# UBC-AWP/vision-sam3-yolo-lameless

Measured on AMD Instinct MI355X. Metric: frames/sec (whole node) for YOLO+SAM3+DINOv3 feature extraction, 1080p clips, higher is better.
Workload: dtype f16; 1 GPU; BASELINE cfg#5, dense schedule: fused per-frame path on a synthetic 5 s @ 30 fps 1080p clip (150 unique BGR frames resident in HBM): YOLOv8-l detect (letterbox 384x640, NMS, scale_boxes; f16 plan) -> SAM (Hiera-B+ image encoder + FPN at 1024x1024, box-prompted mask decoder, 1080p mask + statistics + contour features) + DINOv3 ViT-L/16 embed (224x224) on EVERY frame; per-frame records packed, gathe; parallelism=one clip per GPU, 1 GPU(s), one gather per step, streams=7

## Files before the change

include/lmx.h:

```cpp
#ifndef LMX_H
#define LMX_H
#include <stdint.h>
#ifdef __cplusplus
extern "C" {
#endif

#define LMX_VERSION 100

#define LMX_OK 0
#define LMX_EINVAL (-1)
#define LMX_EHIP (-2)

typedef void* lmx_stream_t;

int lmx_version(void);
const char* lmx_last_error(void);
int lmx_device_count(void);

enum { LMX_F16 = 0, LMX_F32 = 1 };
enum { LMX_ACT_NONE = 0, LMX_ACT_SILU = 1, LMX_ACT_GELU = 2 , LMX_ACT_RELU = 3,
       LMX_ACT_SWIGLU = 4  };

typedef struct {
  const void* A;
// ... 94 lines not shown
                   lmx_stream_t stream);
int lmx_k_upsample2(const void* src, int64_t lds, void* dst, int64_t ldd, int n, int H, int W, int C,
                    lmx_stream_t stream);
int lmx_k_detect_decode(const float* head, int64_t ldh, float* pred, int n, int H, int W, int nc, float stride,
                        int a_off, int A, lmx_stream_t stream);
int lmx_k_scale_boxes(float* boxes, int total, float padx, float pady, float gain, float w, float h,
                      lmx_stream_t stream);

int lmx_k_split3(const float* x, int64_t ldx, int act, const void* res3, int64_t ldr, void* out3, int64_t ldo, int64_t rows,
                 int N, int g, int nsum, int64_t sum_stride, lmx_stream_t stream);
int lmx_k_maxpool5_x3(const void* src3, int64_t lds, void* dst3, int64_t ldd, int n, int H, int W, int C, lmx_stream_t stream);
int lmx_k_stem_conv_x3(const uint8_t* img, const float* w, const float* bias, void* out3, int n, int H, int W, int Cout,
                       lmx_stream_t stream);
int lmx_k_attention_f32(const float* q, int64_t ldq, const float* k, int64_t ldk, const float* v, int64_t ldv, float* o,
                        int64_t ldo, int B, int H, int Tq, int Tk, int hd, float scale, lmx_stream_t stream);
int lmx_k_hyper_mask_f32(const float* up, const float* hyper, float* logits, int n, int G, int C, int act, lmx_stream_t stream);

int lmx_k_pose_gather(const float* raw0, const float* raw1, const float* raw2, int64_t ldk, const int32_t* hw,
                      const float* strides, const int32_t* src, const int32_t* counts, int n, int max_det, int K, int ndim,
                      float padx, float pady, float gain, float w, float h, float* out, lmx_stream_t stream);

int lmx_k_im2col_u8(const uint8_t* img, const float* lut, void* out, int n, int rh, int rw, int IH, int IW, int KH,
                    int KW, int stride, int pad, int64_t ldo, lmx_stream_t stream);
int lmx_k_maxpool2(const void* src, int64_t lds, void* dst, int64_t ldd, int dtype, int n, int H, int W, int C,
                   lmx_stream_t stream);
int lmx_k_cast_f32_f16(const float* src, int64_t lds, void* dst, int64_t ldd, int64_t rows, int cols,
                       lmx_stream_t stream);
int lmx_h_hiera_band(const int* window, const int* q_stride, int n_blocks, int grid, int nh, int nw, int* band);
int lmx_k_band_join(const void* band, const void* table, void* out, int dtype, int n, int H, int Hb, int W, int D,
                    lmx_stream_t stream);

int lmx_k_add_bcast(const void* a, int a_dtype, int64_t lda, const float* b, int64_t ldb, int b_rows, void* out,
                    int out_dtype, int64_t ldo, int64_t rows, int D, lmx_stream_t stream);
int lmx_k_prompt_box(const float* boxes, int64_t ldb, float* sparse, int n, double sx, double sy, float S,
                     const float* gauss, const float* corner, int F, lmx_stream_t stream);
int lmx_k_hyper_mask(const void* up, const float* hyper, float* logits, int n, int G, int C, lmx_stream_t stream);
int lmx_k_mask_post(const float* logits, int n, int L, int T, int nh, int nw, int h, int w, uint8_t* mask,
                    int64_t* stats, float* workspace, lmx_stream_t stream);
int lmx_k_prompt_points(const float* points, const int32_t* labels, int Np, const float* boxes, int64_t ldb, float* sparse, int n,
                        double sx, double sy, float S, const float* gauss, const float* point_embed, const float* not_a_point,
                        const float* corner, int F, lmx_stream_t stream);
#define LMX_MASK_EMBED_PARAMS 4684
int lmx_k_mask_embed(const float* mask_input, const void* emb, int emb_dtype, int64_t lde, const float* params, float* keys,
                     int64_t ldk, int n, int G, lmx_stream_t stream);
int lmx_k_hyper_mask_multi(const void* up, const float* hyper, float* logits, int n, int M, int G, int C, lmx_stream_t stream);
int lmx_k_hyper_mask_multi_f32(const float* up, const float* hyper, float* logits, int n, int M, int G, int C, int act,
// ... 22 lines not shown
```

vision-sam3-yolo-lameless_amd/csrc/pre.hip:

```cpp
#include "common.h"

namespace {

constexpr int PRECISION_BITS = 32 - 8 - 2;

__device__ __forceinline__ uint8_t clip8(int v) {
  v >>= PRECISION_BITS;
  return (uint8_t)(v < 0 ? 0 : (v > 255 ? 255 : v));
}

constexpr int RESIZE_H_MAX_ROW = 16384;
__global__ __launch_bounds__(256) void pil_resize_h_kernel(const uint8_t* __restrict__ src, uint8_t* __restrict__ dst,
                                                           int n, int sh, int sw, int dw,
                                                           const int32_t* __restrict__ bounds,
                                                           const int32_t* __restrict__ kk, int ksize, int swap_rb) {
  __shared__ __attribute__((aligned(16))) uint8_t rowbuf[RESIZE_H_MAX_ROW];
  const int rowb = sw * 3;
  for (int64_t row = blockIdx.x; row < (int64_t)n * sh; row += gridDim.x) {
    const uint8_t* srow = src + row * rowb;
    const int mis = (int)(reinterpret_cast<uintptr_t>(srow) & 15);
    const int head = mis ? 16 - mis : 0;
    for (int i = threadIdx.x; i < head && i < rowb; i += blockDim.x) rowbuf[i] = srow[i];
    const int nvec = (rowb - head) > 0 ? (rowb - head) / 16 : 0;
    for (int v = threadIdx.x; v < nvec; v += blockDim.x) {
      const u32x4 x = *reinterpret_cast<const u32x4*>(srow + head + v * 16);
      uint8_t* d = rowbuf + head + v * 16;
      if ((head & 3) == 0) {
        reinterpret_cast<unsigned*>(d)[0] = x[0];
        reinterpret_cast<unsigned*>(d)[1] = x[1];
        reinterpret_cast<unsigned*>(d)[2] = x[2];
        reinterpret_cast<unsigned*>(d)[3] = x[3];
      } else {
#pragma unroll
        for (int e = 0; e < 16; ++e) d[e] = (uint8_t)(x[e >> 2] >> (8 * (e & 3)));
      }
    }
    for (int i = head + nvec * 16 + threadIdx.x; i < rowb; i += blockDim.x) rowbuf[i] = srow[i];
    __syncthreads();
    uint8_t* drow = dst + row * dw * 3;
    for (int xo = threadIdx.x; xo < dw; xo += blockDim.x) {
      const int xmin = bounds[2 * xo], cnt = bounds[2 * xo + 1];
      const int32_t* k = kk + (int64_t)xo * ksize;
      const uint8_t* s = rowbuf + xmin * 3;
      int a0 = 1 << (PRECISION_BITS - 1), a1 = a0, a2 = a0;
      for (int x = 0; x < cnt; ++x) {
        const int c = k[x];
        a0 += (int)s[3 * x + 0] * c;
        a1 += (int)s[3 * x + 1] * c;
        a2 += (int)s[3 * x + 2] * c;
      }
      uint8_t* d = drow + xo * 3;
      if (swap_rb) {
        d[0] = clip8(a2);
        d[1] = clip8(a1);
        d[2] = clip8(a0);
      } else {
        d[0] = clip8(a0);
        d[1] = clip8(a1);
        d[2] = clip8(a2);
      }
    }
    __syncthreads();
  }
}

__global__ __launch_bounds__(256) void pil_resize_v_kernel(const uint8_t* __restrict__ src, uint8_t* __restrict__ dst,
                                                           int n, int sh, int dh, int w,
                                                           const int32_t* __restrict__ bounds,
                                                           const int32_t* __restrict__ kk, int ksize) {
  const int rowb = w * 3;
  const int64_t total = (int64_t)n * dh * rowb;
  for (int64_t i = (int64_t)blockIdx.x * blockDim.x + threadIdx.x; i < total; i += (int64_t)gridDim.x * blockDim.x) {
    const int xb = (int)(i % rowb);
    const int64_t r = i / rowb;
    const int yo = (int)(r % dh);
    const int img = (int)(r / dh);
    const int ymin = bounds[2 * yo], cnt = bounds[2 * yo + 1];
    const int32_t* k = kk + (int64_t)yo * ksize;
    const uint8_t* s = src + ((int64_t)img * sh + ymin) * rowb + xb;
    int a = 1 << (PRECISION_BITS - 1);
    for (int y = 0; y < cnt; ++y) a += (int)s[(int64_t)y * rowb] * k[y];
    dst[i] = clip8(a);
// ... 154 lines not shown
    if (yo >= dh) break;
    const int py = yo / P, ky = yo - py * P;
    half_t* d = out + (((int64_t)img * gh + py) * gw + px) * ldo + (ky * P + kxp) * 3;
    d[0] = (half_t)(((swap_rb ? acc[r][2] : acc[r][0]) - m0) / s0);
    d[1] = (half_t)((acc[r][1] - m1) / s1);
    d[2] = (half_t)(((swap_rb ? acc[r][0] : acc[r][2]) - m2) / s2);
  }
}

inline int grid_for(int64_t total) {
  int64_t g = (total + 255) / 256;
  if (g > 256 * 8) g = 256 * 8;
  if (g < 1) g = 1;
  return (int)g;
}

}

extern "C" int lmx_k_pil_resize_h(const uint8_t* src, uint8_t* dst, int n, int sh, int sw, int dw, const int32_t* bounds,
                                  const int32_t* kk, int ksize, int swap_rb, lmx_stream_t stream) {
  LMX_REQUIRE(src && dst && bounds && kk, "lmx_k_pil_resize_h: null pointer");
  LMX_REQUIRE(n > 0 && sh > 0 && sw > 0 && dw > 0 && ksize > 0, "lmx_k_pil_resize_h: shape");
  LMX_REQUIRE(sw * 3 <= RESIZE_H_MAX_ROW, "lmx_k_pil_resize_h: source rows wider than %d pixels are not staged", RESIZE_H_MAX_ROW / 3);
  int64_t rows = (int64_t)n * sh;
  hipLaunchKernelGGL(pil_resize_h_kernel, dim3((unsigned)(rows < 256 * 16 ? rows : 256 * 16)), dim3(256), 0,
                     reinterpret_cast<hipStream_t>(stream), src, dst, n, sh, sw, dw, bounds, kk, ksize, swap_rb);
  return lmx_launch_check("pil_resize_h_kernel");
}

extern "C" int lmx_k_pil_resize_v(const uint8_t* src, uint8_t* dst, int n, int sh, int dh, int w, const int32_t* bounds,
                                  const int32_t* kk, int ksize, lmx_stream_t stream) {
  LMX_REQUIRE(src && dst && bounds && kk, "lmx_k_pil_resize_v: null pointer");
  LMX_REQUIRE(n > 0 && sh > 0 && dh > 0 && w > 0 && ksize > 0, "lmx_k_pil_resize_v: shape");
  if ((w * 3) % 4 == 0 && (((uintptr_t)src | (uintptr_t)dst) & 3) == 0) {
    hipLaunchKernelGGL(pil_resize_v4_kernel, dim3(grid_for((int64_t)n * dh * (w * 3 / 4))), dim3(256), 0,
                       reinterpret_cast<hipStream_t>(stream), src, dst, n, sh, dh, w, bounds, kk, ksize);
    return lmx_launch_check("pil_resize_v4_kernel");
  }
  hipLaunchKernelGGL(pil_resize_v_kernel, dim3(grid_for((int64_t)n * dh * w * 3)), dim3(256), 0,
                     reinterpret_cast<hipStream_t>(stream), src, dst, n, sh, dh, w, bounds, kk, ksize);
  return lmx_launch_check("pil_resize_v_kernel");
}

extern "C" int lmx_k_float_resize_patchify(const uint8_t* src, void* out, int n, int sh, int sw, int gh, int gw, int P,
                                           int64_t ldo, const int32_t* bounds_h, const float* kk_h, int ksize_h,
                                           const int32_t* bounds_v, const float* kk_v, int ksize_v, int seg_cols,
                                           float rescale, const float* mean_std, int swap_rb, lmx_stream_t stream) {
  LMX_REQUIRE(src && out && bounds_h && kk_h && bounds_v && kk_v && mean_std, "lmx_k_float_resize_patchify: null pointer");
  LMX_REQUIRE(n > 0 && n <= 65535 && sh > 0 && sw > 0 && gh > 0 && gw > 0 && P > 0 && ksize_h > 0 && ksize_v > 0,
// ... 27 lines not shown
```

vision-sam3-yolo-lameless_amd/lmx/_lib.py:

```python
import ctypes as C
import os

_HERE = os.path.dirname(os.path.abspath(__file__))
LIB_PATH = os.environ.get("LMX_LIB") or os.path.join(_HERE, "liblmx.so")


class LmxError(RuntimeError):
    pass


class GemmDesc(C.Structure):
    _fields_ = [
        ("A", C.c_void_p), ("W", C.c_void_p), ("bias", C.c_void_p), ("scale", C.c_void_p), ("res", C.c_void_p),
        ("C", C.c_void_p),
        ("lda", C.c_int64), ("ldc", C.c_int64), ("ldr", C.c_int64),
        ("M", C.c_int32), ("N", C.c_int32), ("K", C.c_int32),
        ("act", C.c_int32), ("out_dtype", C.c_int32), ("a_mode", C.c_int32),
        ("H", C.c_int32), ("W_", C.c_int32), ("Cin", C.c_int32), ("conv_stride", C.c_int32),
        ("Ho", C.c_int32), ("Wo", C.c_int32), ("res_rows", C.c_int32), ("a_rep", C.c_int32), ("split_k", C.c_int32), ("split_stride", C.c_int64),
        ("ln_out", C.c_void_p), ("ln_gamma", C.c_void_p), ("ln_beta", C.c_void_p), ("ld_ln", C.c_int64), ("ln_eps", C.c_float),
    ]


class AttnDesc(C.Structure):
# ... 30 lines not shown
    "lmx_k_relpos_tables": (_I, [C.POINTER(AttnDesc), _VP, _VP, _I, _VP, _VP]),
    "lmx_k_rope": (_I, [_VP, _I64, _I, _I, _I, _I, _I, _VP, _VP, _VP]),
    "lmx_k_pil_resize_h": (_I, [_VP, _VP, _I, _I, _I, _I, _VP, _VP, _I, _I, _VP]),
    "lmx_k_pil_resize_v": (_I, [_VP, _VP, _I, _I, _I, _I, _VP, _VP, _I, _VP]),
    "lmx_k_patchify_norm": (_I, [_VP, _VP, _I, _I, _I, _I, _I, _I, _I, _I, _I64, _VP, _VP]),
    "lmx_k_float_resize_patchify": (_I, [_VP, _VP, _I, _I, _I, _I, _I, _I, _I64, _VP, _VP, _I, _VP, _VP, _I, _I, _F, _VP, _I, _VP]),
    "lmx_k_assemble_tokens": (_I, [_VP, _VP, _VP, _VP, _I, _I, _I, _I, _VP]),
    "lmx_k_token_mean": (_I, [_VP, _I, _VP, _I, _I, _I, _VP]),
    "lmx_k_swiglu": (_I, [_VP, _I64, _VP, _I64, _I, _I, _VP]),
    "lmx_nms_workspace_bytes": (_I64, [_I, _I]),
    "lmx_k_nms": (_I, [_VP, _I, _I, _I, _F, _D, _I, _F, _VP, _VP, _VP, _VP, _VP, _VP, _VP]),
    "lmx_k_letterbox": (_I, [_VP, _VP, _I, _I, _I, _I, _I, _I, _I, _I, _I, _VP, _VP, _VP, _VP, _I, _VP]),
    "lmx_k_stem_conv": (_I, [_VP, _VP, _VP, _VP, _I, _I, _I, _I, _VP]),
    "lmx_k_split3": (_I, [_VP, _I64, _I, _VP, _I64, _VP, _I64, _I64, _I, _I, _I, _I64, _VP]),
    "lmx_k_maxpool5_x3": (_I, [_VP, _I64, _VP, _I64, _I, _I, _I, _I, _VP]),
    "lmx_k_stem_conv_x3": (_I, [_VP, _VP, _VP, _VP, _I, _I, _I, _I, _VP]),
    "lmx_k_attention_f32": (_I, [_VP, _I64, _VP, _I64, _VP, _I64, _VP, _I64, _I, _I, _I, _I, _I, _F, _VP]),
    "lmx_k_hyper_mask_f32": (_I, [_VP, _VP, _VP, _I, _I, _I, _I, _VP]),
    "lmx_k_maxpool5": (_I, [_VP, _I64, _VP, _I64, _I, _I, _I, _I, _VP]),
    "lmx_k_upsample2": (_I, [_VP, _I64, _VP, _I64, _I, _I, _I, _I, _VP]),
    "lmx_k_detect_decode": (_I, [_VP, _I64, _VP, _I, _I, _I, _I, _F, _I, _I, _VP]),
    "lmx_k_scale_boxes": (_I, [_VP, _I, _F, _F, _F, _F, _F, _VP]),
    "lmx_k_im2col_u8": (_I, [_VP, _VP, _VP, _I, _I, _I, _I, _I, _I, _I, _I, _I, _I64, _VP]),
    "lmx_k_maxpool2": (_I, [_VP, _I64, _VP, _I64, _I, _I, _I, _I, _I, _VP]),
    "lmx_k_cast_f32_f16": (_I, [_VP, _I64, _VP, _I64, _I64, _I, _VP]),
    "lmx_h_hiera_band": (_I, [C.POINTER(C.c_int), C.POINTER(C.c_int), _I, _I, _I, _I, C.POINTER(C.c_int)]),
    "lmx_k_band_join": (_I, [_VP, _VP, _VP, _I, _I, _I, _I, _I, _I, _VP]),
    "lmx_k_add_bcast":(_I, [_VP, _I, _I64, _VP, _I64, _I, _VP, _I, _I64, _I64, _I, _VP]),
    "lmx_h_mask_features": (_I, [_VP, _I, _I, _VP]),
    "lmx_h_iou_matrix": (_I, [_VP, _I, _VP, _I, _VP]),
    "lmx_h_assign": (_I, [_VP, _I, _I, _VP, _VP]),
    "lmx_contour_workspace_bytes": (_I64, [_I, _I, _I]),
    "lmx_k_contour_features": (_I, [_VP, _I, _I, _I, _VP, _VP, _VP]),
    "lmx_k_prompt_box": (_I, [_VP, _I64, _VP, _I, _D, _D, _F, _VP, _VP, _I, _VP]),
    "lmx_k_hyper_mask": (_I, [_VP, _VP, _VP, _I, _I, _I, _VP]),
    "lmx_k_mask_post": (_I, [_VP, _I, _I, _I, _I, _I, _I, _I, _VP, _VP, _VP, _VP]),
    "lmx_k_prompt_points": (_I, [_VP, _VP, _I, _VP, _I64, _VP, _I, _D, _D, _F, _VP, _VP, _VP, _VP, _I, _VP]),
    "lmx_k_mask_embed": (_I, [_VP, _VP, _I, _I64, _VP, _VP, _I64, _I, _I, _VP]),
    "lmx_k_hyper_mask_multi": (_I, [_VP, _VP, _VP, _I, _I, _I, _I, _VP]),
    "lmx_k_hyper_mask_multi_f32": (_I, [_VP, _VP, _VP, _I, _I, _I, _I, _I, _VP]),
    "lmx_k_mask_logits": (_I, [_VP, _I, _I, _I, _I, _I, _I, _I, _VP, _VP]),
    "lmx_k_mask_score": (_I, [_VP, _I, _I, _I, _I, _I, _I, _I, _D, _D, _VP, _VP, _VP]),
    "lmx_k_nms_boxes": (_I, [_VP, _I64, _VP, _VP, _I, _D, _VP, _VP, _VP, _VP]),
}

_lib = None
# ... 26 lines not shown
```

vision-sam3-yolo-lameless_amd/lmx/kernels.py:

```python
import ctypes as C
import os
import threading

import torch

from . import _lib
from ._lib import AttnDesc, GemmDesc, LmxError, check

F16, F32 = 0, 1
ACT_NONE, ACT_SILU, ACT_GELU, ACT_RELU, ACT_SWIGLU = 0, 1, 2, 3, 4
_DT = {torch.float16: F16, torch.float32: F32}


_tls = threading.local()


def _stream(dev):
    _tls.dev = dev
    return C.c_void_p(torch.cuda.current_stream(dev).cuda_stream)


def _ptr(t):
    return C.c_void_p(t.data_ptr()) if t is not None else C.c_void_p(0)

# ... 129 lines not shown
        h, g, b, eps = ln_out
        Mh, Nh, ldh = _rows(h, "gemm ln_out")
        if (Mh, Nh) != (Mout, Nout) or h.dtype != torch.float16:
            raise LmxError(f"gemm: ln_out must be float16 [{Mout},{Nout}], got {h.dtype} {tuple(h.shape)}")
        if any(t.dtype != torch.float32 or t.numel() != Nout or not t.is_contiguous() for t in (g, b)):
            raise LmxError("gemm: ln_out's gamma and beta must be contiguous float32 [N]")
        d.ln_out, d.ln_gamma, d.ln_beta, d.ld_ln, d.ln_eps = h.data_ptr(), g.data_ptr(), b.data_ptr(), ldh, float(eps)
    check(_lib.load().lmx_k_gemm(C.byref(d), _stream(dev)), "lmx_k_gemm")
    return out


def im2col_u8(img, lut, IH, IW, KH, KW, stride, pad, ldo):
    dev = _dev(img, lut)
    n, rh, rw, c = img.shape
    if c != 3 or img.dtype != torch.uint8 or not img.is_contiguous():
        raise LmxError("im2col_u8: img must be contiguous uint8 [n,h,w,3]")
    OH, OW = (IH + 2 * pad - KH) // stride + 1, (IW + 2 * pad - KW) // stride + 1
    out = torch.empty((n * OH * OW, ldo), dtype=torch.float16, device=img.device)
    check(_lib.load().lmx_k_im2col_u8(_ptr(img), _ptr(lut), _ptr(out), n, rh, rw, IH, IW, KH, KW, stride, pad, ldo,
                                      _stream(dev)), "lmx_k_im2col_u8")
    return out


def maxpool2(x, out):
    dev = _dev(x, out)
    n, H, W, Cc, ps = _nhwc(x, "maxpool2 x")
    no, Ho, Wo, Co, pso = _nhwc(out, "maxpool2 out")
    if (no, Ho, Wo, Co) != (n, H // 2, W // 2, Cc) or x.dtype != out.dtype:
        raise LmxError("maxpool2: shape/dtype mismatch")
    check(_lib.load().lmx_k_maxpool2(_ptr(x), ps, _ptr(out), pso, _DT[x.dtype], n, H, W, Cc, _stream(dev)), "lmx_k_maxpool2")
    return out


def cast_f16(x, out=None):
    dev = _dev(x, out)
    rows, cols, lds = _rows(x, "cast src")
    if out is None:
        out = torch.empty((rows, cols), dtype=torch.float16, device=x.device)
    check(_lib.load().lmx_k_cast_f32_f16(_ptr(x), lds, _ptr(out), out.stride(0), rows, cols, _stream(dev)),
          "lmx_k_cast_f32_f16")
    return out


def hiera_band(windows, q_strides, grid, nh, nw):
    nb = len(windows)
    if nb != len(q_strides):
# ... 703 lines not shown
    out = torch.empty((n, 8), dtype=torch.int64, device=mask.device)
    check(lib.lmx_k_contour_features(_ptr(mask), n, h, w, _ptr(out), _ptr(ws), _stream(dev)), "lmx_k_contour_features")
    return out


LAUNCH_TRACE = None
_raw_lib = None
RIDGE_FLOP_PER_BYTE = 2500e12 / 8e12


def _work(name, args):
    if name == "lmx_k_gemm":
        d = args[0]._obj
        M, N, Kd = d.M, d.N, d.K
        osz = 4 if d.out_dtype == F32 else 2
        a_bytes = 2 * M * (Kd // max(d.a_rep, 1))
        if d.a_mode == 1:
            a_bytes = 2 * (M // max(d.Ho * d.Wo, 1)) * d.H * d.W_ * d.Cin
        by = a_bytes + 2 * N * Kd + osz * (M // 4 if d.a_mode == 2 else M) * (N // 2 if d.act == ACT_SWIGLU else N) + (osz * (d.res_rows or M) * N if d.res else 0)
        by += 2 * M * N if d.ln_out else 0
        fl = 2.0 * M * N * Kd
        key = f"gemm M={M} N={N} K={Kd} out={'f32' if osz == 4 else 'f16'} conv3x3={d.a_mode} act={d.act} res={int(bool(d.res))}" + (" ln_out" if d.ln_out else "")
        return ("gemm/mfma-bound" if fl / by >= RIDGE_FLOP_PER_BYTE else "gemm/hbm-bound"), fl, by, key
    if name == "lmx_k_attention":
        d = args[0]._obj
        fl = 4.0 * d.B * d.H * d.Tq * d.Tk * d.hd
        by = 2 * d.H * d.hd * d.B * (2 * d.Tq + 2 * d.Tk)
        key = f"attention B={d.B} H={d.H} Tq={d.Tq} Tk={d.Tk} hd={d.hd} mode={d.mode} ws={d.ws} qs={d.q_stride} rel={int(bool(d.rel))}"
        return ("attention/mfma-bound" if fl / by >= RIDGE_FLOP_PER_BYTE else "attention/hbm-bound"), fl, by, key
    if name == "lmx_k_layernorm":
        in_dt, out_dt, rows, D = args[1], args[6], args[8], args[9]
        return "layernorm", 0.0, rows * D * ((4 if in_dt == F32 else 2) + (4 if out_dt == F32 else 2)), f"layernorm rows={rows} D={D} in={in_dt} out={out_dt}"
    if name == "lmx_k_ln_mlp_img":
        rows, D = args[4], args[5]
        return "fused ln+mlp", 16.0 * D * D * rows, (8 + (2 if args[7] else 0) + (2 if args[8] else 0)) * D * rows, f"ln_mlp_img rows={rows} D={D}"
    if name == "lmx_k_ln_mlp":
        rows, D = args[8], args[9]
        return "fused ln+mlp", 16.0 * D * D * rows, (16 + (2 if args[12] else 0) + (2 if args[15] else 0)) * D * rows, f"ln_mlp rows={rows} D={D}"
    if name == "lmx_k_hiera_attn8":
        n_, Gh, Gw, D = args[10], args[11], args[12], args[13]
        rows = n_ * Gh * Gw
        return "fused attention half", rows * (8.0 * D * D + 256.0 * D), rows * D * (8 + (2 if args[0] else 0)), f"hiera_attn8 rows={rows} D={D} ln_inside={int(not args[0])}"
    if name == "lmx_k_hiera_attn4":
        n_, Gh, Gw, D = args[5], args[6], args[7], args[8]
        rows = n_ * Gh * Gw
        return "fused attention half", rows * (8.0 * D * D + 64.0 * D), rows * D * 10, f"hiera_attn4 rows={rows} D={D}"
# ... 80 lines not shown
```

vision-sam3-yolo-lameless_amd/lmx/sam.py:

```python
import math
import os
import threading
from dataclasses import dataclass

import numpy as np
import torch

from . import kernels as K
from . import resample

SAM_PIXEL_MEAN = (123.675, 116.28, 103.53)
SAM_PIXEL_STD = (58.395, 57.12, 57.375)


@dataclass
class HieraConfig:
    hidden: int = 112
    blocks: tuple = (2, 3, 16, 3)
    dims: tuple = (112, 224, 448, 896)
    heads: tuple = (2, 4, 8, 16)
    windows: tuple = (8, 4, 14, 7)
    global_blocks: tuple = (12, 16, 20)
    pos_bkg: tuple = (14, 14)
    q_pool_stages: int = 3
# ... 189 lines not shown
    kslot = np.array([16 * (2 * s_ + hb) + 4 * g + i for s_ in range(nks) for g in range(4) for hb in range(2) for i in range(4)])
    k15, k7 = (lambda r: r & 15), (lambda r: (r >> 1) & 7)
    imgs = []
    for ch in range(4 * D // 64):
        m1 = np.zeros((64, cols), np.float16)
        ok = kslot < D
        m1[:, ok] = w1[64 * ch: 64 * ch + 64][:, kslot[ok]].astype(np.float16)
        m2 = np.zeros((D, 64), np.float16)
        m2[:, :] = w2[:, 64 * ch + kslot[:64]].astype(np.float16)
        i1, i2 = _lds_image(m1, k15), _lds_image(m2, k7)
        if D <= 128:
            both = i1.copy()
            both[8192:8192 + D * 64] = i2[:D * 64]
            imgs.append(both)
        else:
            imgs += [i1, i2]
    z = np.zeros((D,), np.float32)
    bias = np.concatenate([b1, b2, g2, e2, gn if gn is not None else z, en if en is not None else z]).astype(np.float32)
    return np.stack(imgs), bias


class HieraEncoder:

    def __init__(self, cfg, state_dict, device="cuda", fused_mlp=True, band=True):
        self.cfg = cfg
        self.band = band
        self.device = torch.device(device)
        self.fused_mlp = fused_mlp and not os.environ.get("LMX_NO_FUSED_MLP")
        dev = self.device
        sd = state_dict

        def t32(a):
            return torch.from_numpy(np.ascontiguousarray(a, dtype=np.float32)).to(dev)

        def t16(a):
            return t32(a).to(torch.float16).contiguous()

        w = np.transpose(sd["backbone.patch_embed.projection.weight"], (0, 2, 3, 1)).reshape(cfg.hidden, 147)
        self.k_pad = 152
        self.pe_w = t16(np.concatenate([w, np.zeros((cfg.hidden, self.k_pad - 147), np.float32)], 1))
        self.pe_b = t32(sd["backbone.patch_embed.projection.bias"])
        g = cfg.image // 4
        pe = torch.nn.functional.interpolate(torch.from_numpy(sd["backbone.pos_embed"]), size=(g, g), mode="bicubic")
        win = torch.from_numpy(sd["backbone.pos_embed_window"])
        pe = pe + win.tile([x // y for x, y in zip(pe.shape, win.shape)])
        self.pos = pe.permute(0, 2, 3, 1).reshape(g * g, cfg.hidden).contiguous().to(dev)
        self.grid0 = g
        self.blocks = []
        for i, (dim, dim_out, heads, win_, qs) in enumerate(cfg.block_plan()):
# ... 41 lines not shown
        self._tabs = {}
        self.first_global = next((i for i, B in enumerate(self.blocks) if B["win"] == 0), None)
        self._bands, self._band_tabs, self._band_lock = {}, {}, threading.Lock()

    def _tables(self, h, w):
        key = (h, w)
        if key not in self._tabs:
            nh, nw = resize_longest_side(h, w, self.cfg.image)
            dev = self.device

            def up(tab):
                b, k, ks = tab
                return (torch.from_numpy(b).to(dev), torch.from_numpy(k).to(dev), ks)

            th = up(resample.coeff_tables(w, nw, resample.BILINEAR)) if nw != w else None
            tv = up(resample.coeff_tables(h, nh, resample.BILINEAR)) if nh != h else None
            self._tabs[key] = (nh, nw, th, tv)
        return self._tabs[key]

    def preprocess(self, frames, band=0):
        n, h, w, _ = frames.shape
        nh, nw, th, tv = self._tables(h, w)
        img = K.pil_resize(frames, nw, nh, th, tv, swap_rb=False)
        S = self.cfg.image
        return img, K.im2col_u8(img, self.lut, 4 * band if band else S, S, 7, 7, 4, 3, self.k_pad)

    def band_rows(self, nh, nw):
        if (nh, nw) not in self._bands:
            plan = self.cfg.block_plan()
            self._bands[(nh, nw)] = K.hiera_band([p[3] for p in plan], [p[4] for p in plan], self.grid0, nh, nw)
        return self._bands[(nh, nw)]

    def _selection(self):
        H = W = self.grid0
        sel = []
        for i, B in enumerate(self.blocks[:self.first_global]):
            dim, D, heads, win, qs = B["dim"], B["dim_out"], B["heads"], B["win"], B["qs"]
            sel.append((self._attn8(i, H, W), "attnp" in B and K.hiera_attn_pool_ok(dim, D, heads, win, H, W, qs),
                        "attn4" in B and K.hiera_attn4_ok(D, heads, win, H, W, qs), "mlp_img" in B and K.ln_mlp_img_ok(D, H * W)))
            if qs:
                H, W = H // 2, W // 2
        return tuple(sel)

    def _band_table(self, frames, nh, nw, band):
        key = (nh, nw, band, self._selection())
        tab = self._band_tabs.get(key)
        if tab is not None:
            return tab
        if torch.cuda.is_current_stream_capturing():
            raise K.LmxError("HieraEncoder: the constant rows below the band are not built for this frame geometry, and a stream capture "
                             "cannot build them (it needs a synchronisation): call encode() once before capturing")
        with self._band_lock:
            if key in self._band_tabs:
                return self._band_tabs[key]
            trace, K.LAUNCH_TRACE = K.LAUNCH_TRACE, None
            try:
                g = self.grid0
                x, H, W, stages, stages16 = self.trunk(self.preprocess(frames[:1])[1], 1, until=self.first_global)

                def below(t, Hs, Ws):
                    return t.reshape(Hs, Ws, -1)[band * Hs // g:].reshape(-1, t.shape[-1]).clone()

                tab = dict(x=below(x, H, W), stages=[below(s, *s.shape[1:3]) for s in stages],
                           stages16=[below(s16, *s.shape[1:3]) if s16 is not None else None for s, s16 in zip(stages, stages16)])
            finally:
                K.LAUNCH_TRACE = trace
            torch.cuda.current_stream(self.device).synchronize()
            self._band_tabs[key] = tab
        return tab

    def trunk(self, patches, n, band=0, table=None, lowest=0, until=None):
        cfg = self.cfg
        g = self.grid0
        H, W = band or g, g
        Hf = g
        x = K.gemm(patches, self.pe_w, bias=self.pe_b, res=self.pos[:H * g], res_rows=H * g, out_dtype=torch.float32)
        stage_ends = set(int(v) for v in np.cumsum(cfg.blocks) - 1)
        stages, stages16 = [], []
        dev = x.device
        h_next = None
        for i, B in enumerate(self.blocks):
            if i == until:
                return x, H, W, stages, stages16
            if band and i == self.first_global:
                x = K.band_join(x.view(n, H, W, -1), table["x"], Hf).view(n * Hf * W, -1)
                H, band, h_next = Hf, 0, None
            dim, D, heads, qs = B["dim"], B["dim_out"], B["heads"], B["qs"]
            rows = n * H * W
            h2 = None
            if self._attn8(i, H, W):
                if B["attn8_ln"]:
                    K.hiera_attn8(x, B["attn8"], n, H, W, heads, ln=(B["g1"], B["b1"], cfg.eps))
                else:
                    K.hiera_attn8(x, B["attn8"], n, H, W, heads, h=h_next if h_next is not None else K.layernorm(x, B["g1"], B["b1"], cfg.eps))
            elif "attnp" in B and K.hiera_attn_pool_ok(dim, D, heads, B["win"], H, W, qs):
                x = K.hiera_attn_pool(h_next if h_next is not None else K.layernorm(x, B["g1"], B["b1"], cfg.eps), B["attnp"], n, H, W, heads, D)
                H, W = H // 2, W // 2
            elif "attn4" in B and K.hiera_attn4_ok(D, heads, B["win"], H, W, qs):
                K.hiera_attn4(h_next if h_next is not None else K.layernorm(x, B["g1"], B["b1"], cfg.eps), x, B["attn4"], n, H, W, heads)
# ... 97 lines not shown
            if i not in cfg.fpn_top_down or i == nlev:
                K.gemm(a, w, bias=b, out=out.view(-1, cfg.fpn_dim))
            else:
                up = torch.empty((n, H, W, cfg.fpn_dim), dtype=torch.float16, device=s.device)
                K.upsample2(prev, up)
                K.gemm(a, w, bias=b, res=up.view(-1, cfg.fpn_dim), out=out.view(-1, cfg.fpn_dim))
            prev = out
            feats[i] = out
        return feats[:3]

    def encode_patches(self, patches, n):
        stages, stages16 = self.trunk(patches, n)
        return dict(fpn=self.fpn(stages, stages16), stages=stages)

    def encode(self, frames, precision=None, outputs="all"):
        if outputs not in ("all", "embedding"):
            raise ValueError(f"outputs {outputs!r}: expected 'all' or 'embedding'")
        lowest = 2 if outputs == "embedding" else 0
        n, h, w, _ = frames.shape
        nh, nw = self._tables(h, w)[:2]
        band = self.band_rows(nh, nw) if self.band else 0
        table = self._band_table(frames, nh, nw, band) if band else None
        img, patches = self.preprocess(frames, band)
        stages, stages16 = self.trunk(patches, n, band, table, lowest)
        return dict(fpn=self.fpn(stages, stages16, lowest), stages=stages, resized=img)


@dataclass
class SamVitConfig:
    hidden: int = 768
    layers: int = 12
    heads: int = 12
    mlp: int = 3072
    global_idx: tuple = (2, 5, 8, 11)
    window: int = 14
    patch: int = 16
    image: int = 1024
    out_ch: int = 256
    eps: float = 1e-6

    @property
    def grid(self):
        return self.image // self.patch


def sam_vit_b():
    return SamVitConfig()
# ... 160 lines not shown
```

Measured before the change: 788.2 frames/s.

## Fuse Hiera patch-embed im2col with GEMM and restructure horizontal resize kernel

Measured after the change: 794.0 frames/s (median of 6 runs). About the same (+0.7%).

```diff
diff --git a/include/lmx.h b/include/lmx.h
--- a/include/lmx.h
+++ b/include/lmx.h
@@ -140,6 +140,10 @@
 
 int lmx_k_im2col_u8(const uint8_t* img, const float* lut, void* out, int n, int rh, int rw, int IH, int IW, int KH,
                     int KW, int stride, int pad, int64_t ldo, lmx_stream_t stream);
+int lmx_h_patch_embed_ok(int N, int KH, int KW, int stride, int pad, int* ok);
+int lmx_k_patch_embed_u8(const uint8_t* img, const float* lut, const void* w, const float* bias, const float* res, int64_t ldr,
+                         int res_rows, float* out, int64_t ldc, int n, int rh, int rw, int IH, int IW, int N, int KH, int KW,
+                         int stride, int pad, lmx_stream_t stream);
 int lmx_k_maxpool2(const void* src, int64_t lds, void* dst, int64_t ldd, int dtype, int n, int H, int W, int C,
                    lmx_stream_t stream);
 int lmx_k_cast_f32_f16(const float* src, int64_t lds, void* dst, int64_t ldd, int64_t rows, int cols,
diff --git a/vision-sam3-yolo-lameless_amd/csrc/patch_embed.hip b/vision-sam3-yolo-lameless_amd/csrc/patch_embed.hip
--- /dev/null
+++ b/vision-sam3-yolo-lameless_amd/csrc/patch_embed.hip
@@ -0,0 +1,209 @@
+#include "common.h"
+
+namespace {
+
+constexpr int PE_TOK = 128;
+constexpr int PE_K = 147, PE_LDW = 152;
+constexpr int PE_RS = 168;
+constexpr int PE_ROW_BYTES = (4 * (PE_TOK - 1) + 7) * 3;
+constexpr int PE_P16 = 1554;
+constexpr int PE_LINES = (PE_ROW_BYTES + 15 + 15) / 16;
+constexpr int PE_PF = (7 * PE_LINES + 255) / 256;
+static_assert(PE_P16 >= PE_ROW_BYTES, "normalised row");
+
+struct PeTile {
+  int b, oy, tx0, ntok, y0, xs;
+  bool live;
+};
+__device__ __forceinline__ PeTile pe_tile(int tile, int tpr, int OH, int OW, int rh, int rw) {
+  PeTile t;
+  const int tx = tile % tpr, r = tile / tpr;
+  t.oy = r % OH;
+  t.b = r / OH;
+  t.tx0 = tx * PE_TOK;
+  t.ntok = OW - t.tx0 < PE_TOK ? OW - t.tx0 : PE_TOK;
+  t.y0 = 4 * t.oy - 3;
+  t.xs = 4 * t.tx0 - 3;
+  t.live = t.y0 < rh && t.xs < rw;
+  return t;
+}
+struct PeLine {
+  int ky;
+  intptr_t c0, L, g0, g1;
+  bool row_ok;
+};
+__device__ __forceinline__ PeLine pe_line(const PeTile& t, int item, const uint8_t* img, int rh, int rw) {
+  PeLine l;
+  l.ky = item % 7;
+  const int ci = item / 7;
+  const int y = t.y0 + l.ky;
+  l.row_ok = y >= 0 && y < rh;
+  const int x_lo = t.xs < 0 ? 0 : t.xs;
+  int x_hi = t.xs + 4 * (t.ntok - 1) + 7;
+  x_hi = x_hi < rw ? x_hi : rw;
+  const intptr_t rowp = reinterpret_cast<intptr_t>(img) + ((int64_t)t.b * rh + y) * rw * 3;
+  l.L = rowp + t.xs * 3;
+  l.g0 = rowp + x_lo * 3;
+  l.g1 = rowp + x_hi * 3;
+  l.c0 = (l.L & ~(intptr_t)15) + 16 * ci;
+  return l;
+}
+
+template <int NF>
+__global__ __launch_bounds__(256, 2) void patch_embed_u8_kernel(const uint8_t* __restrict__ img, const float* __restrict__ lut,
+                                                                const half_t* __restrict__ w, const float* __restrict__ bias,
+                                                                const float* __restrict__ res, int64_t ldr, int res_rows,
+                                                                float* __restrict__ out, int64_t ldc, int rh, int rw, int OH, int OW,
+                                                                int ntiles) {
+  __shared__ __attribute__((aligned(16))) half_t patch[PE_TOK * PE_RS];
+  __shared__ __attribute__((aligned(16))) half_t rows16[7 * PE_P16];
+  __shared__ half_t lut_s[768];
+  const int tid = threadIdx.x, lane = tid & 63;
+  const int wave = __builtin_amdgcn_readfirstlane(tid >> 6);
+  const int frow = lane & 15, fq = lane >> 4;
+  for (int i = tid; i < 768; i += 256) lut_s[i] = (half_t)lut[i];
+  for (int i = tid; i < PE_TOK * 3; i += 256) *reinterpret_cast<half8_t*>(patch + (i / 3) * PE_RS + 144 + (i % 3) * 8) = half8_t{0, 0, 0, 0, 0, 0, 0, 0};
+
+  half8_t wf[5][NF];
+#pragma unroll
+  for (int t = 0; t < 5; ++t)
+#pragma unroll
+    for (int j = 0; j < NF; ++j) {
+      const int k0 = 32 * t + 8 * fq;
+      wf[t][j] = half8_t{0, 0, 0, 0, 0, 0, 0, 0};
+      if (k0 < PE_LDW) wf[t][j] = *reinterpret_cast<const half8_t*>(w + (j * 16 + frow) * PE_LDW + k0);
+    }
+
+  const int tpr = (OW + PE_TOK - 1) / PE_TOK;
+  u32x4 pf[PE_PF];
+  auto request = [&](const PeTile& t) {
+    if (!t.live) return;
+#pragma unroll
+    for (int q = 0; q < PE_PF; ++q) {
+      const int item = tid + 256 * q;
+      pf[q] = u32x4{0, 0, 0, 0};
+      if (item < 7 * PE_LINES) {
+        const PeLine l = pe_line(t, item, img, rh, rw);
+        if (l.row_ok && l.c0 + 16 > l.g0 && l.c0 < l.g1) pf[q] = *reinterpret_cast<const u32x4*>(l.c0);
+      }
+    }
+  };
+  if ((int)blockIdx.x < ntiles) request(pe_tile(blockIdx.x, tpr, OH, OW, rh, rw));
+  for (int tile = blockIdx.x; tile < ntiles; tile += gridDim.x) {
+    const PeTile T = pe_tile(tile, tpr, OH, OW, rh, rw);
+    if (T.live) {
+#pragma unroll
+      for (int q = 0; q < PE_PF; ++q) {
+        const int item = tid + 256 * q;
+        if (item < 7 * PE_LINES) {
+          const PeLine l = pe_line(T, item, img, rh, rw);
+          const int i0 = (int)(l.c0 - l.L);
+          half_t* d = rows16 + l.ky * PE_P16;
+#pragma unroll
+          for (int e = 0; e < 16; ++e) {
+            const int i = i0 + e;
+            if (i >= 0 && i < PE_ROW_BYTES) {
+              const unsigned byte = (pf[q][e >> 2] >> (8 * (e & 3))) & 255u;
+              const bool in = l.row_ok && l.c0 + e >= l.g0 && l.c0 + e < l.g1;
+              d[i] = in ? lut_s[(i % 3) * 256 + byte] : (half_t)0.f;
+            }
+          }
+        }
+      }
+      __syncthreads();
+#pragma unroll
+      for (int it = 0; it < PE_TOK * 19 / 256 + 1; ++it) {
+        const int tok = tid & (PE_TOK - 1);
+        const int ck = __builtin_amdgcn_readfirstlane((it * 256 + tid) / PE_TOK);
+        if (ck < 19) {
+          half8_t v;
+#pragma unroll
+          for (int e = 0; e < 8; ++e) {
+            const int k = ck * 8 + e;
+            const int ky = k / 21, j = k - ky * 21;
+            v[e] = k < PE_K ? rows16[ky * PE_P16 + 12 * tok + j] : (half_t)0.f;
+          }
+          *reinterpret_cast<half8_t*>(patch + tok * PE_RS + ck * 8) = v;
+        }
+      }
+      __syncthreads();
+    }
+    if (tile + (int)gridDim.x < ntiles) request(pe_tile(tile + gridDim.x, tpr, OH, OW, rh, rw));
+    const int mbase = T.oy * OW + T.tx0;
+    const int rbase = res_rows > 0 ? (int)(((int64_t)T.b * OH * OW + mbase) % res_rows) : 0;
+#pragma unroll
+    for (int i = 0; i < 2; ++i) {
+      f32x4 acc[NF];
+#pragma unroll
+      for (int j = 0; j < NF; ++j) acc[j] = f32x4{0.f, 0.f, 0.f, 0.f};
+      const int tok = wave * 32 + i * 16 + frow;
+      if (T.live) {
+        const half_t* ap = patch + tok * PE_RS + fq * 8;
+        half8_t af[5];
+#pragma unroll
+        for (int t = 0; t < 5; ++t) af[t] = *reinterpret_cast<const half8_t*>(ap + 32 * t);
+#pragma unroll
+        for (int t = 0; t < 5; ++t)
+#pragma unroll
+          for (int j = 0; j < NF; ++j) acc[j] = __builtin_amdgcn_mfma_f32_16x16x32_f16(wf[t][j], af[t], acc[j], 0, 0, 0);
+      }
+      if (tok < T.ntok) {
+        const int64_t m = (int64_t)T.b * OH * OW + mbase + tok;
+        const int64_t mr = res_rows > 0 ? (int64_t)((rbase + tok) % res_rows) : m;
+        const float* rp = res + mr * ldr + fq * 4;
+        float* op = out + m * ldc + fq * 4;
+#pragma unroll
+        for (int j = 0; j < NF; ++j) {
+          f32x4 v = acc[j];
+          v += *reinterpret_cast<const f32x4*>(bias + j * 16 + fq * 4);
+          f32x4 o = v;
+          o += *reinterpret_cast<const f32x4*>(rp + j * 16);
+          *reinterpret_cast<f32x4*>(op + j * 16) = o;
+        }
+      }
+    }
+  }
+}
+
+template <int NF>
+int launch_patch_embed(const uint8_t* img, const float* lut, const void* w, const float* bias, const float* res, int64_t ldr,
+                       int res_rows, float* out, int64_t ldc, int rh, int rw, int OH, int OW, int ntiles, hipStream_t st) {
+  int dev;
+  LMX_TRY(lmx_stream_device(st, &dev));
+  const int cus = lmx_cu_count(dev);
+  if (cus < 0) return cus;
+  const int grid = ntiles < 2 * cus ? ntiles : 2 * cus;
+  hipLaunchKernelGGL(patch_embed_u8_kernel<NF>, dim3((unsigned)grid), dim3(256), 0, st, img, lut, reinterpret_cast<const half_t*>(w), bias,
+                     res, ldr, res_rows, out, ldc, rh, rw, OH, OW, ntiles);
+  return lmx_launch_check("patch_embed_u8_kernel");
+}
+
+}
+
+extern "C" int lmx_h_patch_embed_ok(int N, int KH, int KW, int stride, int pad, int* ok) {
+  LMX_REQUIRE(ok, "lmx_h_patch_embed_ok: null pointer");
+  *ok = KH == 7 && KW == 7 && stride == 4 && pad == 3 && N % 16 == 0 && N >= 96 && N <= 128;
+  return LMX_OK;
+}
+
+extern "C" int lmx_k_patch_embed_u8(const uint8_t* img, const float* lut, const void* w, const float* bias, const float* res, int64_t ldr,
+                                    int res_rows, float* out, int64_t ldc, int n, int rh, int rw, int IH, int IW, int N, int KH, int KW,
+                                    int stride, int pad, lmx_stream_t stream) {
+  LMX_REQUIRE(img && lut && w && bias && res && out, "lmx_k_patch_embed_u8: null pointer");
+  int ok = 0;
+  LMX_TRY(lmx_h_patch_embed_ok(N, KH, KW, stride, pad, &ok));
+  LMX_REQUIRE(ok, "lmx_k_patch_embed_u8: built for 7 x 7 / stride 4 / pad 3 and N = 96, 112, 128 (lmx_h_patch_embed_ok); got %d x %d / %d / %d, N=%d: "
+              "use lmx_k_im2col_u8 + lmx_k_gemm", KH, KW, stride, pad, N);
+  LMX_REQUIRE(n > 0 && rh > 0 && rw > 0 && rh <= IH && rw <= IW, "lmx_k_patch_embed_u8: geometry");
+  LMX_REQUIRE((int64_t)rh * rw * 3 < 0x7fffffffll, "lmx_k_patch_embed_u8: frame too large");
+  const int OH = (IH + 2 * pad - KH) / stride + 1, OW = (IW + 2 * pad - KW) / stride + 1;
+  const int64_t ntiles = (int64_t)n * OH * ((OW + PE_TOK - 1) / PE_TOK);
+  LMX_REQUIRE((int64_t)n * OH * OW < 0x7fffffffll && ntiles < 0x7fffffffll, "lmx_k_patch_embed_u8: too many tokens");
+  LMX_REQUIRE(res_rows >= 0 && ldr >= N && ldc >= N && ldr % 4 == 0 && ldc % 4 == 0, "lmx_k_patch_embed_u8: ldr=%lld ldc=%lld res_rows=%d",
+              (long long)ldr, (long long)ldc, res_rows);
+  LMX_REQUIRE(aligned16(w) && aligned16(bias) && aligned16(res) && aligned16(out), "lmx_k_patch_embed_u8: w, bias, res and out must be 16-byte aligned");
+  hipStream_t st = reinterpret_cast<hipStream_t>(stream);
+  if (N == 96) return launch_patch_embed<6>(img, lut, w, bias, res, ldr, res_rows, out, ldc, rh, rw, OH, OW, (int)ntiles, st);
+  if (N == 112) return launch_patch_embed<7>(img, lut, w, bias, res, ldr, res_rows, out, ldc, rh, rw, OH, OW, (int)ntiles, st);
+  return launch_patch_embed<8>(img, lut, w, bias, res, ldr, res_rows, out, ldc, rh, rw, OH, OW, (int)ntiles, st);
+}
diff --git a/vision-sam3-yolo-lameless_amd/csrc/pre.hip b/vision-sam3-yolo-lameless_amd/csrc/pre.hip
--- a/vision-sam3-yolo-lameless_amd/csrc/pre.hip
+++ b/vision-sam3-yolo-lameless_amd/csrc/pre.hip
@@ -10,54 +10,143 @@
 }
 
 constexpr int RESIZE_H_MAX_ROW = 16384;
-__global__ __launch_bounds__(256) void pil_resize_h_kernel(const uint8_t* __restrict__ src, uint8_t* __restrict__ dst,
+constexpr int RESIZE_H_SEG = 2048;
+constexpr int RESIZE_H_THREADS = 512;
+constexpr int RESIZE_H_ROWBUF = RESIZE_H_MAX_ROW + 48;
+constexpr int RESIZE_H_OUTBUF = RESIZE_H_SEG * 3 + 16;
+constexpr int RESIZE_H_TAB_MAX = 65536 - RESIZE_H_ROWBUF - RESIZE_H_OUTBUF;
+constexpr int RESIZE_H_PF = RESIZE_H_MAX_ROW / 16 / RESIZE_H_THREADS;
+
+template <bool FAST>
+__device__ __forceinline__ int resize_h_mul(unsigned byte, int c) {
+  return FAST ? __mul24((int)byte, c) : (int)byte * c;
+}
+template <bool FAST>
+__device__ __forceinline__ void resize_h_pixel(const uint8_t* rowbuf, int o, int cnt, const int32_t* k, int& a0, int& a1, int& a2) {
+  const unsigned* wp = reinterpret_cast<const unsigned*>(rowbuf + (o & ~3));
+  const unsigned sh = (unsigned)o & 3u;
+  for (int x = 0; x < cnt; x += 4, wp += 3) {
+    const unsigned r0 = wp[0], r1 = wp[1], r2 = wp[2], r3 = wp[3];
+    const unsigned w0 = __builtin_amdgcn_alignbyte(r1, r0, sh), w1 = __builtin_amdgcn_alignbyte(r2, r1, sh),
+                   w2 = __builtin_amdgcn_alignbyte(r3, r2, sh);
+    const int c0 = k[x];
+    const int c1 = x + 1 < cnt ? k[x + 1] : 0, c2 = x + 2 < cnt ? k[x + 2] : 0, c3 = x + 3 < cnt ? k[x + 3] : 0;
+    a0 += resize_h_mul<FAST>(w0 & 255u, c0);
+    a1 += resize_h_mul<FAST>((w0 >> 8) & 255u, c0);
+    a2 += resize_h_mul<FAST>((w0 >> 16) & 255u, c0);
+    a0 += resize_h_mul<FAST>(w0 >> 24, c1);
+    a1 += resize_h_mul<FAST>(w1 & 255u, c1);
+    a2 += resize_h_mul<FAST>((w1 >> 8) & 255u, c1);
+    a0 += resize_h_mul<FAST>((w1 >> 16) & 255u, c2);
+    a1 += resize_h_mul<FAST>(w1 >> 24, c2);
+    a2 += resize_h_mul<FAST>(w2 & 255u, c2);
+    a0 += resize_h_mul<FAST>((w2 >> 8) & 255u, c3);
+    a1 += resize_h_mul<FAST>((w2 >> 16) & 255u, c3);
+    a2 += resize_h_mul<FAST>(w2 >> 24, c3);
+  }
+}
+
+template <bool TAB>
+__global__ __launch_bounds__(RESIZE_H_THREADS) void pil_resize_h_kernel(const uint8_t* __restrict__ src, uint8_t* __restrict__ dst,
                                                            int n, int sh, int sw, int dw,
                                                            const int32_t* __restrict__ bounds,
                                                            const int32_t* __restrict__ kk, int ksize, int swap_rb) {
-  __shared__ __attribute__((aligned(16))) uint8_t rowbuf[RESIZE_H_MAX_ROW];
+  extern __shared__ __attribute__((aligned(16))) uint8_t resize_h_smem[];
+  uint8_t* rowbuf = resize_h_smem;
+  uint8_t* outbuf = resize_h_smem + RESIZE_H_ROWBUF;
+  const int32_t* bnd = bounds;
+  const int32_t* kks = kk;
+  bool fast = false;
+  if (TAB) {
+    int32_t* tab = reinterpret_cast<int32_t*>(resize_h_smem + RESIZE_H_ROWBUF + RESIZE_H_OUTBUF);
+    for (int i = threadIdx.x; i < 2 * dw; i += blockDim.x) tab[i] = bounds[i];
+    int wide = 0;
+    for (int i = threadIdx.x; i < dw * ksize; i += blockDim.x) {
+      const int c = kk[i];
+      tab[2 * dw + i] = c;
+      wide |= (unsigned)(c + (1 << 23)) >= (1u << 24);
+    }
+    bnd = tab;
+    kks = tab + 2 * dw;
+    fast = !__syncthreads_or(wide);
+  }
+  const int tid = threadIdx.x;
   const int rowb = sw * 3;
-  for (int64_t row = blockIdx.x; row < (int64_t)n * sh; row += gridDim.x) {
+  const int64_t rows = (int64_t)n * sh;
+  u32x4 pf[RESIZE_H_PF];
+  unsigned pfb = 0;
+  auto request = [&](int64_t row) {
     const uint8_t* srow = src + row * rowb;
     const int mis = (int)(reinterpret_cast<uintptr_t>(srow) & 15);
-    const int head = mis ? 16 - mis : 0;
-    for (int i = threadIdx.x; i < head && i < rowb; i += blockDim.x) rowbuf[i] = srow[i];
-    const int nvec = (rowb - head) > 0 ? (rowb - head) / 16 : 0;
-    for (int v = threadIdx.x; v < nvec; v += blockDim.x) {
-      const u32x4 x = *reinterpret_cast<const u32x4*>(srow + head + v * 16);
-      uint8_t* d = rowbuf + head + v * 16;
-      if ((head & 3) == 0) {
-        reinterpret_cast<unsigned*>(d)[0] = x[0];
-        reinterpret_cast<unsigned*>(d)[1] = x[1];
-        reinterpret_cast<unsigned*>(d)[2] = x[2];
-        reinterpret_cast<unsigned*>(d)[3] = x[3];
-      } else {
-#pragma unroll
-        for (int e = 0; e < 16; ++e) d[e] = (uint8_t)(x[e >> 2] >> (8 * (e & 3)));
+    int head = mis ? 16 - mis : 0;
+    head = head < rowb ? head : rowb;
+    const int nvec = (rowb - head) / 16;
+    const int tail = head + nvec * 16;
+#pragma unroll
+    for (int q = 0; q < RESIZE_H_PF; ++q) {
+      const int v = tid + q * RESIZE_H_THREADS;
+      if (v < nvec) pf[q] = *reinterpret_cast<const u32x4*>(srow + head + v * 16);
+    }
+    if (tid < head) pfb = srow[tid];
+    if (tid >= 16 && tid < 16 + rowb - tail) pfb = srow[tail + tid - 16];
+  };
+  auto commit = [&](int64_t row) -> int {
+    const uint8_t* srow = src + row * rowb;
+    const int mis = (int)(reinterpret_cast<uintptr_t>(srow) & 15);
+    int head = mis ? 16 - mis : 0;
+    head = head < rowb ? head : rowb;
+    const int nvec = (rowb - head) / 16;
+    const int tail = head + nvec * 16;
+    uint8_t* r = rowbuf + mis;
+#pragma unroll
+    for (int q = 0; q < RESIZE_H_PF; ++q) {
+      const int v = tid + q * RESIZE_H_THREADS;
+      if (v < nvec) *reinterpret_cast<u32x4*>(r + head + v * 16) = pf[q];
+    }
+    if (tid < head) r[tid] = (uint8_t)pfb;
+    if (tid >= 16 && tid < 16 + rowb - tail) r[tail + tid - 16] = (uint8_t)pfb;
+    return mis;
+  };
+  int64_t row = blockIdx.x;
+  if (row < rows) request(row);
+  for (; row < rows; row += gridDim.x) {
+    const int mis = commit(row);
+    __syncthreads();
+    if (row + gridDim.x < rows) request(row + gridDim.x);
+    for (int x0 = 0; x0 < dw; x0 += RESIZE_H_SEG) {
+      const int npx = dw - x0 < RESIZE_H_SEG ? dw - x0 : RESIZE_H_SEG;
+      uint8_t* drow = dst + (row * dw + x0) * 3;
+      const int omis = (int)(reinterpret_cast<uintptr_t>(drow) & 15);
+      if (x0) __syncthreads();
+      for (int xl = tid; xl < npx; xl += blockDim.x) {
+        const int xo = x0 + xl;
+        const int xmin = bnd[2 * xo], cnt = bnd[2 * xo + 1];
+        const int32_t* k = kks + (int64_t)xo * ksize;
+        int a0 = 1 << (PRECISION_BITS - 1), a1 = a0, a2 = a0;
+        if (fast)
+          resize_h_pixel<true>(rowbuf, mis + xmin * 3, cnt, k, a0, a1, a2);
+        else
+          resize_h_pixel<false>(rowbuf, mis + xmin * 3, cnt, k, a0, a1, a2);
+        uint8_t* d = outbuf + omis + xl * 3;
+        if (swap_rb) {
+          d[0] = clip8(a2);
+          d[1] = clip8(a1);
+          d[2] = clip8(a0);
+        } else {
+          d[0] = clip8(a0);
+          d[1] = clip8(a1);
+          d[2] = clip8(a2);
+        }
       }
-    }
-    for (int i = head + nvec * 16 + threadIdx.x; i < rowb; i += blockDim.x) rowbuf[i] = srow[i];
-    __syncthreads();
-    uint8_t* drow = dst + row * dw * 3;
-    for (int xo = threadIdx.x; xo < dw; xo += blockDim.x) {
-      const int xmin = bounds[2 * xo], cnt = bounds[2 * xo + 1];
-      const int32_t* k = kk + (int64_t)xo * ksize;
-      const uint8_t* s = rowbuf + xmin * 3;
-      int a0 = 1 << (PRECISION_BITS - 1), a1 = a0, a2 = a0;
-      for (int x = 0; x < cnt; ++x) {
-        const int c = k[x];
-        a0 += (int)s[3 * x + 0] * c;
-        a1 += (int)s[3 * x + 1] * c;
-        a2 += (int)s[3 * x + 2] * c;
-      }
-      uint8_t* d = drow + xo * 3;
-      if (swap_rb) {
-        d[0] = clip8(a2);
-        d[1] = clip8(a1);
-        d[2] = clip8(a0);
-      } else {
-        d[0] = clip8(a0);
-        d[1] = clip8(a1);
-        d[2] = clip8(a2);
+      __syncthreads();
+      const int end = omis + npx * 3;
+      for (int c = tid; c * 16 < end; c += blockDim.x) {
+        const int lo = c * 16;
+        if (lo >= omis && lo + 16 <= end) {
+          *reinterpret_cast<u32x4*>(drow - omis + lo) = *reinterpret_cast<const u32x4*>(outbuf + lo);
+        } else {
+          for (int e = lo < omis ? omis : lo; e < lo + 16 && e < end; ++e) drow[e - omis] = outbuf[e];
+        }
       }
     }
     __syncthreads();
@@ -258,9 +347,21 @@
   LMX_REQUIRE(src && dst && bounds && kk, "lmx_k_pil_resize_h: null pointer");
   LMX_REQUIRE(n > 0 && sh > 0 && sw > 0 && dw > 0 && ksize > 0, "lmx_k_pil_resize_h: shape");
   LMX_REQUIRE(sw * 3 <= RESIZE_H_MAX_ROW, "lmx_k_pil_resize_h: source rows wider than %d pixels are not staged", RESIZE_H_MAX_ROW / 3);
-  int64_t rows = (int64_t)n * sh;
-  hipLaunchKernelGGL(pil_resize_h_kernel, dim3((unsigned)(rows < 256 * 16 ? rows : 256 * 16)), dim3(256), 0,
-                     reinterpret_cast<hipStream_t>(stream), src, dst, n, sh, sw, dw, bounds, kk, ksize, swap_rb);
+  const int64_t rows = (int64_t)n * sh;
+  hipStream_t st = reinterpret_cast<hipStream_t>(stream);
+  const int64_t tab_bytes = (int64_t)dw * (2 + ksize) * 4;
+  if (tab_bytes <= RESIZE_H_TAB_MAX) {
+    int dev;
+    LMX_TRY(lmx_stream_device(st, &dev));
+    const int cus = lmx_cu_count(dev);
+    if (cus < 0) return cus;
+    const int64_t cap = 3 * (int64_t)cus;
+    hipLaunchKernelGGL(pil_resize_h_kernel<true>, dim3((unsigned)(rows < cap ? rows : cap)), dim3(RESIZE_H_THREADS),
+                       (size_t)(RESIZE_H_ROWBUF + RESIZE_H_OUTBUF + tab_bytes), st, src, dst, n, sh, sw, dw, bounds, kk, ksize, swap_rb);
+  } else {
+    hipLaunchKernelGGL(pil_resize_h_kernel<false>, dim3((unsigned)(rows < 256 * 16 ? rows : 256 * 16)), dim3(RESIZE_H_THREADS),
+                       (size_t)(RESIZE_H_ROWBUF + RESIZE_H_OUTBUF), st, src, dst, n, sh, sw, dw, bounds, kk, ksize, swap_rb);
+  }
   return lmx_launch_check("pil_resize_h_kernel");
 }
 
diff --git a/vision-sam3-yolo-lameless_amd/lmx/_lib.py b/vision-sam3-yolo-lameless_amd/lmx/_lib.py
--- a/vision-sam3-yolo-lameless_amd/lmx/_lib.py
+++ b/vision-sam3-yolo-lameless_amd/lmx/_lib.py
@@ -76,6 +76,8 @@
     "lmx_k_detect_decode": (_I, [_VP, _I64, _VP, _I, _I, _I, _I, _F, _I, _I, _VP]),
     "lmx_k_scale_boxes": (_I, [_VP, _I, _F, _F, _F, _F, _F, _VP]),
     "lmx_k_im2col_u8": (_I, [_VP, _VP, _VP, _I, _I, _I, _I, _I, _I, _I, _I, _I, _I64, _VP]),
+    "lmx_h_patch_embed_ok": (_I, [_I, _I, _I, _I, _I, C.POINTER(C.c_int)]),
+    "lmx_k_patch_embed_u8": (_I, [_VP, _VP, _VP, _VP, _VP, _I64, _I, _VP, _I64, _I, _I, _I, _I, _I, _I, _I, _I, _I, _I, _VP]),
     "lmx_k_maxpool2": (_I, [_VP, _I64, _VP, _I64, _I, _I, _I, _I, _I, _VP]),
     "lmx_k_cast_f32_f16": (_I, [_VP, _I64, _VP, _I64, _I64, _I, _VP]),
     "lmx_h_hiera_band": (_I, [C.POINTER(C.c_int), C.POINTER(C.c_int), _I, _I, _I, _I, C.POINTER(C.c_int)]),
diff --git a/vision-sam3-yolo-lameless_amd/lmx/kernels.py b/vision-sam3-yolo-lameless_amd/lmx/kernels.py
--- a/vision-sam3-yolo-lameless_amd/lmx/kernels.py
+++ b/vision-sam3-yolo-lameless_amd/lmx/kernels.py
@@ -175,6 +175,35 @@
     return out
 
 
+def patch_embed_ok(N, KH, KW, stride, pad):
+    ok = C.c_int(0)
+    check(_lib.load().lmx_h_patch_embed_ok(N, KH, KW, stride, pad, C.byref(ok)), "lmx_h_patch_embed_ok")
+    return bool(ok.value)
+
+
+def patch_embed_u8(img, lut, IH, IW, w, bias, res, res_rows=0, KH=7, KW=7, stride=4, pad=3):
+    dev = _dev(img, lut, w, bias, res)
+    if img.dim() != 4 or img.shape[3] != 3 or img.dtype != torch.uint8 or not img.is_contiguous():
+        raise LmxError("patch_embed_u8: img must be contiguous uint8 [n,h,w,3]")
+    n, rh, rw, _ = img.shape
+    N, Kw, ldw = _rows(w, "patch_embed_u8 W")
+    if w.dtype != torch.float16 or Kw != 152 or ldw != 152:
+        raise LmxError(f"patch_embed_u8: W must be contiguous float16 [N,152], got {w.dtype} {tuple(w.shape)}")
+    if lut.dtype != torch.float32 or lut.numel() != 768 or not lut.is_contiguous():
+        raise LmxError("patch_embed_u8: lut must be contiguous float32 [3,256]")
+    if bias.dtype != torch.float32 or bias.numel() != N or not bias.is_contiguous():
+        raise LmxError("patch_embed_u8: bias must be contiguous float32 [N]")
+    OH, OW = (IH + 2 * pad - KH) // stride + 1, (IW + 2 * pad - KW) // stride + 1
+    M = n * OH * OW
+    Mr, Nr, ldr = _rows(res, "patch_embed_u8 res")
+    if (Mr, Nr) != ((res_rows or M), N) or res.dtype != torch.float32:
+        raise LmxError(f"patch_embed_u8: res must be float32 [{res_rows or M},{N}], got {res.dtype} {tuple(res.shape)}")
+    out = torch.empty((M, N), dtype=torch.float32, device=img.device)
+    check(_lib.load().lmx_k_patch_embed_u8(_ptr(img), _ptr(lut), _ptr(w), _ptr(bias), _ptr(res), ldr, res_rows, _ptr(out), N, n, rh, rw,
+                                           IH, IW, N, KH, KW, stride, pad, _stream(dev)), "lmx_k_patch_embed_u8")
+    return out
+
+
 def maxpool2(x, out):
     dev = _dev(x, out)
     n, H, W, Cc, ps = _nhwc(x, "maxpool2 x")
@@ -924,6 +953,12 @@
         fl = 2.0 * M * N * Kd
         key = f"gemm M={M} N={N} K={Kd} out={'f32' if osz == 4 else 'f16'} conv3x3={d.a_mode} act={d.act} res={int(bool(d.res))}" + (" ln_out" if d.ln_out else "")
         return ("gemm/mfma-bound" if fl / by >= RIDGE_FLOP_PER_BYTE else "gemm/hbm-bound"), fl, by, key
+    if name == "lmx_k_patch_embed_u8":
+        res_rows, n_, rh, rw, IH, IW, N = args[6], args[9], args[10], args[11], args[12], args[13], args[14]
+        M = n_ * ((IH - 1) // 4 + 1) * ((IW - 1) // 4 + 1)
+        fl = 2.0 * M * N * 152
+        by = 3 * n_ * rh * rw + 2 * N * 152 + 4 * (res_rows or M) * N + 4 * M * N
+        return ("gemm/mfma-bound" if fl / by >= RIDGE_FLOP_PER_BYTE else "gemm/hbm-bound"), fl, by, f"patch_embed_u8 M={M} N={N} K=152 out=f32 img={n_}x{rh}x{rw}"
     if name == "lmx_k_attention":
         d = args[0]._obj
         fl = 4.0 * d.B * d.H * d.Tq * d.Tk * d.hd
diff --git a/vision-sam3-yolo-lameless_amd/lmx/sam.py b/vision-sam3-yolo-lameless_amd/lmx/sam.py
--- a/vision-sam3-yolo-lameless_amd/lmx/sam.py
+++ b/vision-sam3-yolo-lameless_amd/lmx/sam.py
@@ -235,9 +235,10 @@
 
 class HieraEncoder:
 
-    def __init__(self, cfg, state_dict, device="cuda", fused_mlp=True, band=True):
+    def __init__(self, cfg, state_dict, device="cuda", fused_mlp=True, band=True, direct_embed=True):
         self.cfg = cfg
         self.band = band
+        self.direct_embed = direct_embed and K.patch_embed_ok(cfg.hidden, 7, 7, 4, 3)
         self.device = torch.device(device)
         self.fused_mlp = fused_mlp and not os.environ.get("LMX_NO_FUSED_MLP")
         dev = self.device
@@ -325,8 +326,13 @@
         n, h, w, _ = frames.shape
         nh, nw, th, tv = self._tables(h, w)
         img = K.pil_resize(frames, nw, nh, th, tv, swap_rb=False)
+        if self.direct_embed:
+            return img, None
+        return img, self.patches(img, band)
+
+    def patches(self, img, band=0):
         S = self.cfg.image
-        return img, K.im2col_u8(img, self.lut, 4 * band if band else S, S, 7, 7, 4, 3, self.k_pad)
+        return K.im2col_u8(img, self.lut, 4 * band if band else S, S, 7, 7, 4, 3, self.k_pad)
 
     def band_rows(self, nh, nw):
         if (nh, nw) not in self._bands:
@@ -359,7 +365,8 @@
             trace, K.LAUNCH_TRACE = K.LAUNCH_TRACE, None
             try:
                 g = self.grid0
-                x, H, W, stages, stages16 = self.trunk(self.preprocess(frames[:1])[1], 1, until=self.first_global)
+                img, patches = self.preprocess(frames[:1])
+                x, H, W, stages, stages16 = self.trunk(patches if patches is not None else (img, 0), 1, until=self.first_global)
 
                 def below(t, Hs, Ws):
                     return t.reshape(Hs, Ws, -1)[band * Hs // g:].reshape(-1, t.shape[-1]).clone()
@@ -377,7 +384,14 @@
         g = self.grid0
         H, W = band or g, g
         Hf = g
-        x = K.gemm(patches, self.pe_w, bias=self.pe_b, res=self.pos[:H * g], res_rows=H * g, out_dtype=torch.float32)
+        if isinstance(patches, tuple):
+            img, img_band = patches
+            if img_band != band:
+                raise K.LmxError(f"HieraEncoder.trunk: frames embedded for band {img_band}, trunk asked for band {band}")
+            S = cfg.image
+            x = K.patch_embed_u8(img, self.lut, 4 * band if band else S, S, self.pe_w, self.pe_b, self.pos[:H * g], res_rows=H * g)
+        else:
+            x = K.gemm(patches, self.pe_w, bias=self.pe_b, res=self.pos[:H * g], res_rows=H * g, out_dtype=torch.float32)
         stage_ends = set(int(v) for v in np.cumsum(cfg.blocks) - 1)
         stages, stages16 = [], []
         dev = x.device
@@ -521,7 +535,7 @@
         band = self.band_rows(nh, nw) if self.band else 0
         table = self._band_table(frames, nh, nw, band) if band else None
         img, patches = self.preprocess(frames, band)
-        stages, stages16 = self.trunk(patches, n, band, table, lowest)
+        stages, stages16 = self.trunk(patches if patches is not None else (img, band), n, band, table, lowest)
         return dict(fpn=self.fpn(stages, stages16, lowest), stages=stages, resized=img)
 
 
```
